# mstksg/tensor-ops

Measured on AMD Instinct MI355X. Metric: gradTOp steps/sec (ffLayer MNIST 784->256->10) + gmul TFLOP/s vs roofline, higher is better.
Workload: dtype f32

## Files before the change

### tensor-ops_amd/csrc/gemm_t32.hip

```cpp
#include <cstdio>
#include <type_traits>

#include "common.hpp"
#include "arg_fit.hpp"

namespace to {

typedef float f32x16 __attribute__((ext_vector_type(16)));
typedef float f32x4 __attribute__((ext_vector_type(4)));

struct T32Args {
  const float* A;
  const float* B;
  long a_sx, b_sx;
  int M, N, K;
  int tiles_m, tiles_n;
  int lgm, lgn;
  unsigned wmag0, wmag1;
  int pd;
  float* C;
  const float* Cin;
  const float* bias;
  const float* dact;
  float* rowsum;
  const float* rowsum_in;
  unsigned long long* dbg;
  long c_sm;
  int gm, gn;
  int act, dact_kind;
  int rowsum_acc;
  float alpha, beta;
  float rowsum_alpha;
};

__device__ __forceinline__ void t32_pin_hot(const T32Args& g) {
  asm volatile("" ::"s"(g.A), "s"(g.B), "s"(g.a_sx), "s"(g.b_sx), "s"(g.M), "s"(g.N), "s"(g.K), "s"(g.tiles_m), "s"(g.tiles_n),
               "s"(g.lgm), "s"(g.lgn), "s"(g.wmag0), "s"(g.wmag1), "s"(g.pd));
}

__device__ __attribute__((aligned(16))) float g_t32_zero[4] = {0.f, 0.f, 0.f, 0.f};

constexpr int T32_BK = 32, T32_NS = 2, T32_NW = 4;
constexpr int T32_CTR = 4096;
constexpr int T32_STAGE = 2 * 32 * T32_BK;
constexpr int T32_WAVE = T32_NS * T32_STAGE;

__device__ __forceinline__ bool t32_tile_of(const T32Args& g, int bid, int& tm, int& tn) {
  const int x = bid & 7, local = bid >> 3, xm = x >> g.lgn, xn = x & ((1 << g.lgn) - 1);
  const int r0 = (g.tiles_m * xm) >> g.lgm, r1 = (g.tiles_m * (xm + 1)) >> g.lgm;
  const int c0 = (g.tiles_n * xn) >> g.lgn, c1 = (g.tiles_n * (xn + 1)) >> g.lgn;
  const int w = c1 - c0;
  if (w <= 0 || local >= (r1 - r0) * w) return false;
  const unsigned mag = w == (g.tiles_n >> g.lgn) ? g.wmag0 : g.wmag1;
  const int q = w == 1 ? local : (int)__umulhi((unsigned)local, mag);
  tm = r0 + q;
  tn = c0 + local - q * w;
  return true;
}

__device__ __forceinline__ int t32_key(int x) { return (x >> 1) & 7; }

template <bool AKC, bool BKC, bool ARAG = false, bool WT = false, int NW = T32_NW, int NS = T32_NS, bool EARLY = false, bool REGU = false, bool PIN = true>
__device__ __forceinline__ int gemm_t32_body(const T32Args& g, const int bid, float* smem) {
  static_assert(!REGU || (NW == 8 && NS == 1 && EARLY && !ARAG), "the register unit belongs to the eight-wave, one-stage, early-DMA form");
  constexpr int WAVE_F = NS * T32_STAGE;
  static_assert(WAVE_F >= 1024 + 64, "a wave's stage memory holds its partial tile and its row sums");
  static_assert(!ARAG || !AKC, "the dword form is for a row-contiguous A");
  constexpr int NA = ARAG ? 16 : 4, PER = NA + 4;
#ifdef TOPS_AB_KNOBS
  const unsigned long long t_entry = __builtin_amdgcn_s_memrealtime();
#endif
  if constexpr (PIN) t32_pin_hot(g);
  const int tid = threadIdx.x, lane = tid & 63;
  const int wave = __builtin_amdgcn_readfirstlane(tid >> 6);
  const int l31 = lane & 31, half = lane >> 5;
#ifdef TOPS_AB_KNOBS
  unsigned long long* dbg = nullptr;
  unsigned long long* wdbg = nullptr;
  auto stamp = [&](int i) { if (dbg) dbg[i] = __builtin_amdgcn_s_memrealtime(); };
  auto stamp_first = [&] {
    const bool mine = g.dbg && (bid == 0 || bid == (int)gridDim.x - 1);
    dbg = (mine && tid == 0) ? g.dbg + (bid == 0 ? 0 : 8) : nullptr;
    wdbg = (mine && lane == 0 && wave < 8) ? g.dbg + 16 + (bid == 0 ? 0 : 16) + 2 * wave : nullptr;
    if (dbg) { dbg[0] = t_entry; dbg[6] = __builtin_amdgcn_s_memrealtime(); }
  };
#else
  auto stamp = [](int) {};
  auto stamp_first = [] {};
#endif
#ifdef TOPS_AB_KNOBS
#define T32_WSTAMP(i) do { if (wdbg) wdbg[i] = __builtin_amdgcn_s_memrealtime(); } while (0)
#else
#define T32_WSTAMP(i) do { } while (0)
#endif
  int tile_m, tile_n;
  if (!t32_tile_of(g, bid, tile_m, tile_n)) return -1;
  const int m0 = tile_m * 32, n0 = tile_n * 32;

  const int erow = tid >> 3, ec4 = (tid & 7) * 4;
  const long grow = m0 + erow, gcol = n0 + ec4;
  const bool evalid = (NW == 4 || tid < 256) && grow < g.M && gcol < g.N;
  f32x4 pf_ci = {0.f, 0.f, 0.f, 0.f}, pf_hd = {0.f, 0.f, 0.f, 0.f}, pf_bias = {0.f, 0.f, 0.f, 0.f};
  auto prefetch_epilogue = [&] {
    if (evalid) {
      if (g.Cin) pf_ci = *reinterpret_cast<const f32x4*>(g.Cin + grow * g.c_sm + gcol);
      if (g.dact) pf_hd = *reinterpret_cast<const f32x4*>(g.dact + grow * g.c_sm + gcol);
      if (g.bias) pf_bias = *reinterpret_cast<const f32x4*>(g.bias + gcol);
    }
  };
  if constexpr (!EARLY) prefetch_epilogue();

  const int U = (g.K + 15) / 16;
  const int k0 = (int)((unsigned)(U * wave) / (unsigned)NW) * 16;
  int k1 = (int)((unsigned)(U * (wave + 1)) / (unsigned)NW) * 16;
  if (k1 > g.K) k1 = g.K;
  int kd = k1;
  bool ru = false;
  if constexpr (REGU) {
    const int nU = (k1 - k0 + 15) / 16;
    ru = (nU & 1) != 0;
    if (ru) kd = k0 + (nU - 1) * 16;
  }
  const int nC = kd > k0 ? (kd - k0 + T32_BK - 1) / T32_BK : 0;

  typedef __attribute__((address_space(3))) void* lptr_t;
  float* wsm = smem + wave * WAVE_F;
  const unsigned lds_w = __builtin_amdgcn_readfirstlane((unsigned)(unsigned long)(lptr_t)wsm);

  const int lr = lane >> 3, ls = lane & 7;
  unsigned oa[4], ob[4];
  bool xa_ok = true, xb_ok = true;
#pragma unroll
  for (int p = 0; p < 4; ++p) {
    if constexpr (AKC) {
      long x = m0 + 8 * p + lr;
      if (x >= g.M) x = g.M - 1;
      oa[p] = (unsigned)((x * g.a_sx + 4 * (ls ^ t32_key(8 * p + lr))) * 4);
    } else {
      oa[p] = (unsigned)(((long)(8 * p + lr) * g.a_sx + m0 + 4 * ls) * 4);
    }
    if constexpr (BKC) {
      long x = n0 + 8 * p + lr;
      if (x >= g.N) x = g.N - 1;
      ob[p] = (unsigned)((x * g.b_sx + 4 * (ls ^ t32_key(8 * p + lr))) * 4);
    } else {
      ob[p] = (unsigned)(((long)(8 * p + lr) * g.b_sx + n0 + 4 * ls) * 4);
    }
  }
  if constexpr (!AKC) xa_ok = m0 + 4 * ls + 3 < g.M;
  if constexpr (!BKC) xb_ok = n0 + 4 * ls + 3 < g.N;
  const bool interior = !ARAG && (AKC || m0 + 32 <= g.M) && (BKC || n0 + 32 <= g.N);
  const long step_a = AKC ? T32_BK * 4L : T32_BK * g.a_sx * 4L, step_b = BKC ? T32_BK * 4L : T32_BK * g.b_sx * 4L;
  const char* sa = reinterpret_cast<const char*>(g.A) + (AKC ? (long)k0 * 4 : (long)k0 * g.a_sx * 4);
  const char* sb = reinterpret_cast<const char*>(g.B) + (BKC ? (long)k0 * 4 : (long)k0 * g.b_sx * 4);

#define T32_DMA(OFF, BASE) asm volatile("global_load_lds_dwordx4 %0, %1 offset:0" ::"v"(OFF), "s"(BASE) : "memory")
#define T32_DMA_V(PTR) asm volatile("global_load_lds_dwordx4 %0, off offset:0" ::"v"(PTR) : "memory")
  const long a_sx_l = g.a_sx;
  const int M_l = g.M;
  auto issue = [&, a_sx_l, M_l](int c) {
    const int seq = c;
    const int kc = k0 + c * T32_BK;
    const unsigned st = lds_w + (unsigned)(seq % NS) * (T32_STAGE * 4);
    const char* ba = sa + (long)c * step_a;
    const char* bb = sb + (long)c * step_b;
    const bool full = kc + T32_BK <= kd;
    if (full && interior) {
#pragma unroll
      for (int p = 0; p < 4; ++p) {
        asm volatile("s_mov_b32 m0, %0\n\ts_nop 0" ::"s"(st + p * 1024) : "memory");
        T32_DMA(oa[p], ba);
      }
#pragma unroll
      for (int p = 0; p < 4; ++p) {
        asm volatile("s_mov_b32 m0, %0\n\ts_nop 0" ::"s"(st + 4096 + p * 1024) : "memory");
        T32_DMA(ob[p], bb);
      }
    } else {
      const char* zero = reinterpret_cast<const char*>(g_t32_zero);
      if constexpr (ARAG) {
#pragma unroll
        for (int e = 0; e < 16; ++e) {
          const int kl = 2 * e + half;
          const bool ok = kc + kl < kd && m0 + l31 < M_l;
          const char* src = ok ? ba + ((long)kl * a_sx_l + m0 + l31) * 4 : zero;
          asm volatile("s_mov_b32 m0, %0\n\ts_nop 0" ::"s"(st + e * 256) : "memory");
          asm volatile("global_load_lds_dword %0, off offset:0" ::"v"(src) : "memory");
        }
      } else {
#pragma unroll
        for (int p = 0; p < 4; ++p) {
          const bool ok = AKC ? (kc + 4 * (ls ^ t32_key(8 * p + lr)) < kd) : (kc + 8 * p + lr < kd && xa_ok);
          const char* src = ok ? ba + oa[p] : zero;
          asm volatile("s_mov_b32 m0, %0\n\ts_nop 0" ::"s"(st + p * 1024) : "memory");
          T32_DMA_V(src);
        }
      }
#pragma unroll
      for (int p = 0; p < 4; ++p) {
        const bool ok = BKC ? (kc + 4 * (ls ^ t32_key(8 * p + lr)) < kd) : (kc + 8 * p + lr < kd && xb_ok);
        const char* src = ok ? bb + ob[p] : zero;
        asm volatile("s_mov_b32 m0, %0\n\ts_nop 0" ::"s"(st + 4096 + p * 1024) : "memory");
        T32_DMA_V(src);
      }
    }
  };
#undef T32_DMA
#undef T32_DMA_V

  f32x16 acc;
#pragma unroll
  for (int r = 0; r < 16; ++r) acc[r] = 0.f;
  float asum = 0.f;
  bool want_rs;

  const int PD = g.pd < NS ? g.pd : NS;
  const int pro = nC < PD ? nC : PD;
  f32x4 ua4[2], ub4[2];
  float ua1[8], ub1[8];
  if constexpr (REGU) {
    if (ru) {
      const float* zero = g_t32_zero;
#pragma unroll
      for (int i = 0; i < 2; ++i) {
        const int kq = kd + 4 * (2 * i + half);
        if constexpr (AKC) {
          long x = m0 + l31;
          if (x >= g.M) x = g.M - 1;
          const float* src = kq < k1 ? g.A + x * g.a_sx + kq : zero;
          asm volatile("global_load_dwordx4 %0, %1, off" : "=&v"(ua4[i]) : "v"(src) : "memory");
        } else {
#pragma unroll
          for (int j = 0; j < 4; ++j) {
            const float* src = (kq + j < k1 && m0 + l31 < g.M) ? g.A + (long)(kq + j) * g.a_sx + m0 + l31 : zero;
            asm volatile("global_load_dword %0, %1, off" : "=&v"(ua1[4 * i + j]) : "v"(src) : "memory");
          }
        }
        if constexpr (BKC) {
          long x = n0 + l31;
          if (x >= g.N) x = g.N - 1;
          const float* src = kq < k1 ? g.B + x * g.b_sx + kq : zero;
          asm volatile("global_load_dwordx4 %0, %1, off" : "=&v"(ub4[i]) : "v"(src) : "memory");
        } else {
#pragma unroll
          for (int j = 0; j < 4; ++j) {
            const float* src = (kq + j < k1 && n0 + l31 < g.N) ? g.B + (long)(kq + j) * g.b_sx + n0 + l31 : zero;
            asm volatile("global_load_dword %0, %1, off" : "=&v"(ub1[4 * i + j]) : "v"(src) : "memory");
          }
        }
      }
    }
    __builtin_amdgcn_sched_barrier(0);
  }
  if constexpr (EARLY) {
    if (pro > 0) issue(0);
    __builtin_amdgcn_sched_barrier(0);
    stamp_first();
    want_rs = g.rowsum != nullptr && tile_n == 0;
    if constexpr (REGU) {
      if (ru) {
        if (pro > 0) asm volatile("s_waitcnt vmcnt(%0)" ::"n"(PER) : "memory");
        else asm volatile("s_waitcnt vmcnt(0)" ::: "memory");
        float fu[8], gu[8];
        if constexpr (AKC) {
          asm volatile("" : "+v"(ua4[0]), "+v"(ua4[1]) :: "memory");
#pragma unroll
          for (int i = 0; i < 2; ++i) { fu[4 * i] = ua4[i].x; fu[4 * i + 1] = ua4[i].y; fu[4 * i + 2] = ua4[i].z; fu[4 * i + 3] = ua4[i].w; }
        } else {
          asm volatile("" : "+v"(ua1[0]), "+v"(ua1[1]), "+v"(ua1[2]), "+v"(ua1[3]), "+v"(ua1[4]), "+v"(ua1[5]), "+v"(ua1[6]), "+v"(ua1[7]) :: "memory");
#pragma unroll
          for (int q = 0; q < 8; ++q) fu[q] = ua1[q];
        }
        if constexpr (BKC) {
          asm volatile("" : "+v"(ub4[0]), "+v"(ub4[1]) :: "memory");
#pragma unroll
          for (int i = 0; i < 2; ++i) { gu[4 * i] = ub4[i].x; gu[4 * i + 1] = ub4[i].y; gu[4 * i + 2] = ub4[i].z; gu[4 * i + 3] = ub4[i].w; }
        } else {
          asm volatile("" : "+v"(ub1[0]), "+v"(ub1[1]), "+v"(ub1[2]), "+v"(ub1[3]), "+v"(ub1[4]), "+v"(ub1[5]), "+v"(ub1[6]), "+v"(ub1[7]) :: "memory");
#pragma unroll
          for (int q = 0; q < 8; ++q) gu[q] = ub1[q];
        }
        __builtin_amdgcn_sched_barrier(0);
#pragma unroll
        for (int q = 0; q < 8; ++q) {
          acc = __builtin_amdgcn_mfma_f32_32x32x2f32(fu[q], gu[q], acc, 0, 0, 0);
          if (want_rs) asum += fu[q];
        }
      }
      __builtin_amdgcn_sched_barrier(0);
    }
    prefetch_epilogue();
    __builtin_amdgcn_sched_barrier(0);
    for (int c = 1; c < pro; ++c) issue(c);
  } else {
    for (int c = 0; c < pro; ++c) issue(c);
    stamp_first();
    want_rs = g.rowsum != nullptr && tile_n == 0;
  }
  stamp(1);

  auto wait_landed = [&](int c) {
    const int newer = (nC - 1 - c) < (PD - 1) ? (nC - 1 - c) : (PD - 1);
    static_assert(3 * PER <= 63, "vmcnt is six bits");
    if (newer >= 3) asm volatile("s_waitcnt vmcnt(%0)" ::"n"(3 * PER) : "memory");
    else if (newer == 2) asm volatile("s_waitcnt vmcnt(%0)" ::"n"(2 * PER) : "memory");
    else if (newer == 1) asm volatile("s_waitcnt vmcnt(%0)" ::"n"(PER) : "memory");
    else asm volatile("s_waitcnt vmcnt(0)" ::: "memory");
  };
  auto steps_of = [&](int c) { return (kd - (k0 + c * T32_BK)) > 16 ? 4 : 2; };
  auto read_frags = [&](int c, float (&fa)[16], float (&fb)[16]) {
    const float* sp = wsm + (c % NS) * T32_STAGE;
    const int nI = steps_of(c);
#pragma unroll
    for (int i = 0; i < 4; ++i) {
      if (i < nI) {
        if constexpr (AKC) {
          const f32x4 v = *reinterpret_cast<const f32x4*>(sp + l31 * 32 + 4 * ((2 * i + half) ^ t32_key(l31)));
          fa[4 * i] = v.x; fa[4 * i + 1] = v.y; fa[4 * i + 2] = v.z; fa[4 * i + 3] = v.w;
        } else {
#pragma unroll
          for (int j = 0; j < 4; ++j) fa[4 * i + j] = sp[(4 * (2 * i + half) + j) * 32 + l31];
        }
        if constexpr (BKC) {
          const f32x4 v = *reinterpret_cast<const f32x4*>(sp + 1024 + l31 * 32 + 4 * ((2 * i + half) ^ t32_key(l31)));
          fb[4 * i] = v.x; fb[4 * i + 1] = v.y; fb[4 * i + 2] = v.z; fb[4 * i + 3] = v.w;
        } else {
#pragma unroll
          for (int j = 0; j < 4; ++j) fb[4 * i + j] = sp[1024 + (4 * (2 * i + half) + j) * 32 + l31];
        }
      }
    }
  };
  auto mma = [&](int c, const float (&fa)[16], const float (&fb)[16]) {
    const int nI = steps_of(c);
#pragma unroll
    for (int i = 0; i < 4; ++i) {
      if (i < nI) {
#pragma unroll
        for (int j = 0; j < 4; ++j) {
          acc = __builtin_amdgcn_mfma_f32_32x32x2f32(fa[4 * i + j], fb[4 * i + j], acc, 0, 0, 0);
          if (want_rs) asum += fa[4 * i + j];
        }
      }
    }
  };
  float fa[16], fb[16];
  for (int c = 0; c < nC; ++c) {
    wait_landed(c);
    if (c == 0) stamp(2);
    read_frags(c, fa, fb);
    asm volatile("s_waitcnt lgkmcnt(0)" ::: "memory");
    __builtin_amdgcn_sched_barrier(0);
    if (c + PD < nC) issue(c + PD);
    __builtin_amdgcn_sched_barrier(0);
    mma(c, fa, fb);
  }
  asm volatile("s_waitcnt vmcnt(0)" ::: "memory");
  stamp(3);
  T32_WSTAMP(0);

#pragma unroll
  for (int r = 0; r < 16; ++r) wsm[((r & 3) + 8 * (r >> 2) + 4 * half) * 32 + l31] = acc[r];
  if (want_rs) wsm[1024 + lane] = asum;
  T32_WSTAMP(1);
  __syncthreads();
  stamp(4);
  f32x4 s = {0.f, 0.f, 0.f, 0.f};
  if (NW == 4 || tid < 256) {
    s = *reinterpret_cast<const f32x4*>(smem + erow * 32 + ec4);
#pragma unroll
    for (int w = 1; w < NW; ++w) s += *reinterpret_cast<const f32x4*>(smem + w * WAVE_F + erow * 32 + ec4);
  }
  if (evalid) {
    f32x4 v = s * g.alpha;
    if (g.Cin) v += pf_ci * g.beta;
    if (g.bias) v += pf_bias;
    if (g.act == 1) {
      v.x = 1.f / (1.f + __expf(-v.x)); v.y = 1.f / (1.f + __expf(-v.y));
      v.z = 1.f / (1.f + __expf(-v.z)); v.w = 1.f / (1.f + __expf(-v.w));
    } else if (g.act == 2) {
      v.x = tanhf(v.x); v.y = tanhf(v.y); v.z = tanhf(v.z); v.w = tanhf(v.w);
    }
    if (g.dact) {
      if (g.dact_kind == 0) v *= pf_hd * (1.f - pf_hd);
      else v *= 1.f - pf_hd * pf_hd;
    }
    if constexpr (WT) {
      typedef unsigned int u32x4 __attribute__((ext_vector_type(4)));
      const u32x4 u = {__float_as_uint(v.x), __float_as_uint(v.y), __float_as_uint(v.z), __float_as_uint(v.w)};
      float* dst = g.C + grow * g.c_sm + gcol;
      asm volatile("global_store_dwordx4 %0, %1, off sc0 sc1" ::"v"(dst), "v"(u) : "memory");
    } else {
      *reinterpret_cast<f32x4*>(g.C + grow * g.c_sm + gcol) = v;
    }
  }
  if (want_rs && tid < 32) {
    const long m = m0 + tid;
    if (m < g.M) {
      float t = 0.f;
#pragma unroll
      for (int w = 0; w < NW; ++w) t += smem[w * WAVE_F + 1024 + tid] + smem[w * WAVE_F + 1024 + 32 + tid];
      if (g.rowsum_acc) g.rowsum[m] = (g.rowsum_in ? g.rowsum_in[m] : g.rowsum[m]) + g.rowsum_alpha * t;
      else g.rowsum[m] = t;
    }
  }
  stamp(5);
#undef T32_WSTAMP
  return tile_m;
}

struct T32HeadArgs {
  const float* W2;
  const float* bias2;
  const float* target;
  float* dz;
  float* loss_out;
  float* tail_out;
  unsigned* ctr;
  int* status;
  long w_sn, dz_sm;
  int N2, loss_rows;
  float alpha2;
};

__global__ __launch_bounds__(256) void gemm_t32_head_kernel(T32Args g, T32HeadArgs h) {
  extern __shared__ __attribute__((aligned(1024))) float t32_smem[];
  const int tid = threadIdx.x, lane = tid & 63;
  const int wave = __builtin_amdgcn_readfirstlane(tid >> 6);
  const unsigned long long t_entry = g.dbg ? __builtin_amdgcn_s_memrealtime() : 0ull;
  int tile_m, tile_n;
  if (!t32_tile_of(g, (int)blockIdx.x, tile_m, tile_n)) return;
  const long grow = (long)tile_m * 32 + 4 * tile_n + wave;
  const bool rv = grow < g.M;
  f32x4 w4[16];
#pragma unroll
  for (int n = 0; n < 16; ++n) {
    w4[n] = f32x4{0.f, 0.f, 0.f, 0.f};
    if (n < h.N2) w4[n] = *reinterpret_cast<const f32x4*>(h.W2 + (long)n * h.w_sn + 4 * lane);
  }
  const float b_l = (lane < h.N2 && h.bias2) ? h.bias2[lane] : 0.f;
  const float t_l = (lane < h.N2 && rv) ? h.target[grow * h.dz_sm + lane] : 0.f;

  gemm_t32_body<true, true, false, true>(g, (int)blockIdx.x, t32_smem);

  unsigned long long* const hd = (g.dbg && tid == 0 && blockIdx.x == 0) ? g.dbg + 8 : nullptr;
  asm volatile("s_waitcnt vmcnt(0)" ::: "memory");
  __syncthreads();
  __shared__ int gave_up;
  if (tid == 0) {
    unsigned* arrive = h.ctr + tile_m;
    __hip_atomic_fetch_add(arrive, 1u, __ATOMIC_RELAXED, __HIP_MEMORY_SCOPE_AGENT);
    if (hd) { hd[0] = t_entry; hd[1] = __builtin_amdgcn_s_memrealtime(); hd[7] = 1; }
    const unsigned long long t0 = __builtin_amdgcn_s_memrealtime();
    int bad = 0;
    while (__hip_atomic_load(arrive, __ATOMIC_RELAXED, __HIP_MEMORY_SCOPE_AGENT) < (unsigned)g.tiles_n) {
      __builtin_amdgcn_s_sleep(2);
      if (__builtin_amdgcn_s_memrealtime() - t0 > 200000000ull) {
        bad = 1;
        break;
      }
    }
    gave_up = bad;
    if (bad && h.status) *h.status = tile_m + 1;
  }
  __syncthreads();
  if (gave_up) return;
  if (hd) hd[2] = __builtin_amdgcn_s_memrealtime();

  typedef unsigned int u32x4 __attribute__((ext_vector_type(4)));
  f32x4 h4 = {0.f, 0.f, 0.f, 0.f};
  if (rv) {
    u32x4 u;
    const float* src = g.C + grow * g.c_sm + 4 * lane;
    asm volatile("global_load_dwordx4 %0, %1, off sc0 sc1\n\ts_waitcnt vmcnt(0)" : "=v"(u) : "v"(src) : "memory");
    h4 = f32x4{__uint_as_float(u.x), __uint_as_float(u.y), __uint_as_float(u.z), __uint_as_float(u.w)};
  }
  float z[16];
#pragma unroll
  for (int n = 0; n < 16; ++n) {
    z[n] = 0.f;
    if (n < h.N2) {
      z[n] = h4.x * w4[n].x + h4.y * w4[n].y + h4.z * w4[n].z + h4.w * w4[n].w;
#pragma unroll
      for (int off = 1; off < 64; off <<= 1) z[n] += __shfl_xor(z[n], off, 64);
    }
  }
  float v = -INFINITY;
#pragma unroll
  for (int n = 0; n < 16; ++n)
    if (n < h.N2 && lane == n) v = z[n] * h.alpha2 + b_l;
  auto sum16 = [](float x) {
#pragma unroll
    for (int off = 8; off > 0; off >>= 1) x += __shfl_xor(x, off, 64);
    return x;
  };
  const bool lv = lane < h.N2;
  float out_l, loss_l;
  if (h.loss_rows == 1) {
    float mx = v;
#pragma unroll
    for (int off = 8; off > 0; off >>= 1) mx = fmaxf(mx, __shfl_xor(mx, off, 64));
    const float e = lv ? expf(v - mx) : 0.f;
    const float se = sum16(e), sy = sum16(t_l);
    const float pr = e / se;
    out_l = lv ? pr * sy - t_l : 0.f;
    loss_l = lv ? -t_l * logf(pr) : 0.f;
  } else {
    const float sg = 1.f / (1.f + expf(-v));
    const float e = t_l - sg;
    out_l = lv ? -2.f * e * sg * (1.f - sg) : 0.f;
    loss_l = lv ? e * e : 0.f;
  }
  if (rv) {
    if (lv) h.dz[grow * h.dz_sm + lane] = out_l;
    if (h.loss_out) {
      const float l = sum16(loss_l);
      if (lane == 0) h.loss_out[grow] = l;
    }
  }
  if (hd) hd[3] = __builtin_amdgcn_s_memrealtime();
  if (h.tail_out) {
    f32x4 a = {0.f, 0.f, 0.f, 0.f};
#pragma unroll
    for (int n = 0; n < 16; ++n)
      if (n < h.N2) {
        const float d = __shfl(out_l, n, 64);
        a += w4[n] * d;
      }
    if (rv) *reinterpret_cast<f32x4*>(h.tail_out + grow * 256 + 4 * lane) = a * h4 * (1.f - h4);
  }
  if (hd) hd[4] = __builtin_amdgcn_s_memrealtime();
  __syncthreads();
  if (tid == 0) {
    unsigned* leave = h.ctr + T32_CTR + tile_m;
    const unsigned seen = __hip_atomic_fetch_add(leave, 1u, __ATOMIC_RELAXED, __HIP_MEMORY_SCOPE_AGENT);
    if (seen == (unsigned)(g.tiles_n - 1)) {
      __hip_atomic_store(h.ctr + tile_m, 0u, __ATOMIC_RELAXED, __HIP_MEMORY_SCOPE_AGENT);
      __hip_atomic_store(leave, 0u, __ATOMIC_RELAXED, __HIP_MEMORY_SCOPE_AGENT);
    }
  }
}

__host__ __device__ __forceinline__ int t32_tiles(int extent) { return (extent + 31) >> 5; }
__host__ __device__ __forceinline__ unsigned t32_pack_map(int lgm, int lgn, int pd) { return (unsigned)lgm | ((unsigned)lgn << 8) | ((unsigned)pd << 16); }

template <bool AKC, bool BKC, int NW = T32_NW, int NS = T32_NS, bool EARLY = false, bool REGU = false>
__global__ __launch_bounds__(NW * 64) void gemm_t32_kernel(const float* A, const float* B, int a_sx, int b_sx, int M, int N, int K,
                                                           unsigned map, unsigned wmag0, unsigned wmag1, T32Args cold) {
  extern __shared__ __attribute__((aligned(1024))) float t32_smem[];
  T32Args g = cold;
  g.A = A; g.B = B;
  g.a_sx = a_sx; g.b_sx = b_sx;
  g.M = M; g.N = N; g.K = K;
  g.tiles_m = t32_tiles(M); g.tiles_n = t32_tiles(N);
  g.lgm = (int)(map & 255u); g.lgn = (int)((map >> 8) & 255u); g.pd = (int)(map >> 16);
  g.wmag0 = wmag0; g.wmag1 = wmag1;
  gemm_t32_body<AKC, BKC, false, false, NW, NS, EARLY, REGU, false>(g, (int)blockIdx.x, t32_smem);
}

template <bool ARAG2>
__global__ __launch_bounds__(256) void gemm_t32_pair_kernel(T32Args g1, T32Args g2, int n1) {
  extern __shared__ __attribute__((aligned(1024))) float t32_smem[];
  if ((int)blockIdx.x < n1) gemm_t32_body<false, false, false>(g1, (int)blockIdx.x, t32_smem);
  else gemm_t32_body<false, false, ARAG2>(g2, (int)blockIdx.x - n1, t32_smem);
}

static bool t32_plan_map(T32Args& g) {
  if ((long)g.tiles_m * g.tiles_n > 65535) return false;
  auto lg = [](int v) { int l = 0; while ((1 << l) < v) ++l; return l; };
  auto mag = [](int w) { return w >= 2 ? (unsigned)((0xFFFFFFFFull / (unsigned)w) + 1ull) : 0u; };
  g.lgm = lg(g.gm);
  g.lgn = lg(g.gn);
  const int wlo = g.tiles_n >> g.lgn;
  g.wmag0 = mag(wlo);
  g.wmag1 = mag(wlo + 1);
  return true;
}

static bool t32_fill(const GemmProblem& p, T32Args& g, bool& akc, bool& bkc, bool allow_ragged_a = false, bool* ragged_a = nullptr) {
  if (p.dtype != TO_F32 || p.batch != 1 || p.reduce_batch) return false;
  if (p.loss_rows || p.tail_out || p.loss_out) return false;
  akc = p.a_sk == 1 && p.K > 1;
  bkc = p.b_sk == 1 && p.K > 1;
  if (!akc && p.a_sm != 1) return false;
  if (!bkc && p.b_sn != 1) return false;
  if (p.K % 4 != 0 || p.N % 4 != 0) return false;
  const bool rag = !akc && (p.M % 4 != 0 || p.a_sk % 4 != 0 || (reinterpret_cast<uintptr_t>(p.A) & 15u));
  if (ragged_a) *ragged_a = rag;
  if (rag && !allow_ragged_a) return false;
  if (akc && p.a_sm % 4 != 0) return false;
  if (bkc && p.b_sn % 4 != 0) return false;
  if (!bkc && p.b_sk % 4 != 0) return false;
  if ((reinterpret_cast<uintptr_t>(p.A) & 3u) || ((akc || !rag) && (reinterpret_cast<uintptr_t>(p.A) & 15u))) return false;
  if ((reinterpret_cast<uintptr_t>(p.B) | reinterpret_cast<uintptr_t>(p.C)) & 15u) return false;
  if (p.c_sm % 4 != 0) return false;
  if (p.Cin && (reinterpret_cast<uintptr_t>(p.Cin) & 15u)) return false;
  if (p.dact && (reinterpret_cast<uintptr_t>(p.dact) & 15u)) return false;
  if (p.bias && (reinterpret_cast<uintptr_t>(p.bias) & 15u)) return false;
  if (p.beta != 0.0 && !p.Cin) return false;
  if (p.act > 2) return false;
  if (!t32_spans_fit(p.M, p.N, p.K, p.a_sm, p.a_sk, p.b_sn, p.b_sk)) return false;
  g.A = (const float*)p.A; g.B = (const float*)p.B; g.C = (float*)p.C;
  g.Cin = p.beta != 0.0 ? (const float*)p.Cin : nullptr;
  g.M = (int)p.M; g.N = (int)p.N; g.K = (int)p.K;
  g.a_sx = akc ? p.a_sm : p.a_sk;
  g.b_sx = bkc ? p.b_sn : p.b_sk;
  g.c_sm = p.c_sm;
  g.tiles_m = t32_tiles((int)p.M); g.tiles_n = t32_tiles((int)p.N);
  {
    int best = 1 << 30;
    for (int gm : {8, 4, 2, 1}) {
      const int gn = 8 / gm;
      const int cost = (g.tiles_m + gm - 1) / gm + (g.tiles_n + gn - 1) / gn;
      if (cost < best) { best = cost; g.gm = gm; g.gn = gn; }
    }
  }
  if (!t32_plan_map(g)) return false;
  g.alpha = (float)p.alpha; g.beta = (float)p.beta;
  g.bias = (const float*)p.bias; g.dact = (const float*)p.dact; g.act = p.act; g.dact_kind = p.dact_kind;
  g.rowsum = (float*)p.rowsum; g.rowsum_in = (const float*)p.rowsum_in; g.rowsum_alpha = (float)p.rowsum_alpha;
  g.rowsum_acc = p.rowsum_acc ? 1 : 0;
  static const int pd = [] { const char* e = ab_getenv("TOPS_T32_PD"); const int v = e ? atoi(e) : 2; return v < 1 ? 1 : (v > T32_NS ? T32_NS : v); }();
  g.pd = pd;
  static unsigned long long* dbg = [] {
    unsigned long long* p = nullptr;
    if (ab_getenv("TOPS_T32_STAMPS") && hipHostMalloc(reinterpret_cast<void**>(&p), 48 * sizeof(unsigned long long), hipHostMallocMapped) == hipSuccess) {
      for (int i = 0; i < 48; ++i) p[i] = 0;
      static unsigned long long* keep = p;
      atexit([] {
        if (keep[15]) {
          const unsigned long long* k = keep + 8;
          std::fprintf(stderr, "[t32] joined launch, workgroup 0, us since it began: its tile stored and arrived %.2f, all eight tiles of the row block "
                               "there %.2f, loss head of its four rows done %.2f, tail stored %.2f (entered %.2f us after stamp 0)\n",
                       (k[1] - k[0]) * 0.01, (k[2] - k[0]) * 0.01, (k[3] - k[0]) * 0.01, (k[4] - k[0]) * 0.01, ((double)k[0] - (double)keep[0]) * 0.01);
        }
        for (int w = 0; w < (keep[15] ? 1 : 2); ++w) {
          const unsigned long long* k = keep + 8 * w;
          std::fprintf(stderr, "[t32] %s workgroup of the last launch, us since its first instruction: first operand load out %.2f, prologue DMA issued %.2f, "
                               "first chunk landed %.2f, K loop done %.2f, partials met %.2f, done %.2f; began %.2f us after workgroup 0\n", w ? "last" : "first",
                       (k[6] - k[0]) * 0.01, (k[1] - k[0]) * 0.01, (k[2] - k[0]) * 0.01, (k[3] - k[0]) * 0.01, (k[4] - k[0]) * 0.01, (k[5] - k[0]) * 0.01,
                       ((double)k[0] - (double)keep[0]) * 0.01);
          const unsigned long long* wv = keep + 16 + 16 * w;
          std::fprintf(stderr, "[t32]   per wave, K loop done / partial written:");
          for (int q = 0; q < 8; ++q)
            if (wv[2 * q]) std::fprintf(stderr, "  w%d %.2f / %.2f", q, ((double)wv[2 * q] - (double)k[0]) * 0.01, ((double)wv[2 * q + 1] - (double)k[0]) * 0.01);
          std::fprintf(stderr, "\n");
        }
      });
    }
    return p;
  }();
  g.dbg = dbg;
  return true;
}

bool gemm_t32_applicable(const GemmProblem& p) {
  static const int enable = [] { const char* e = ab_getenv("TOPS_GEMM_T32"); return e ? atoi(e) : 1; }();
  if (!enable) return false;
  T32Args g;
  bool akc, bkc;
  if (!t32_fill(p, g, akc, bkc)) return false;
  const long tiles = (long)g.tiles_m * g.tiles_n;
  static const long max_tiles = [] { const char* e = ab_getenv("TOPS_T32_MAXTILES"); return e ? atol(e) : 512L; }();
  return tiles >= 96 && tiles <= max_tiles && p.K >= 256 && p.K <= 8192;
}

bool launch_gemm_t32_pair(const GemmProblem& p1, const GemmProblem& p2, hipStream_t s, bool dry);

static long t32_grid(const T32Args& g) {
  const long rm = (g.tiles_m + g.gm - 1) / g.gm, rn = (g.tiles_n + g.gn - 1) / g.gn;
  return 8 * rm * rn;
}

static void t32_attr(const void* k) { TO_HIP(hipFuncSetAttribute(k, hipFuncAttributeMaxDynamicSharedMemorySize, T32_NW * T32_WAVE * 4)); }

constexpr int T32_W8_DEFAULT = 1;
constexpr int T32_W8_NS = 1;
constexpr bool T32_EARLY = true;
constexpr bool T32_REGU = true;

template <int NW, int NS, bool EARLY, bool REGU = false>
static void t32_launch_nw(const T32Args& g, bool akc, bool bkc, hipStream_t s) {
  constexpr size_t lds = (size_t)NW * NS * T32_STAGE * 4;
  static bool attr = false;
  if (!attr) {
    TO_HIP(hipFuncSetAttribute(reinterpret_cast<const void*>(gemm_t32_kernel<true, true, NW, NS, EARLY, REGU>), hipFuncAttributeMaxDynamicSharedMemorySize, (int)lds));
    TO_HIP(hipFuncSetAttribute(reinterpret_cast<const void*>(gemm_t32_kernel<true, false, NW, NS, EARLY, REGU>), hipFuncAttributeMaxDynamicSharedMemorySize, (int)lds));
    TO_HIP(hipFuncSetAttribute(reinterpret_cast<const void*>(gemm_t32_kernel<false, true, NW, NS, EARLY, REGU>), hipFuncAttributeMaxDynamicSharedMemorySize, (int)lds));
    TO_HIP(hipFuncSetAttribute(reinterpret_cast<const void*>(gemm_t32_kernel<false, false, NW, NS, EARLY, REGU>), hipFuncAttributeMaxDynamicSharedMemorySize, (int)lds));
    attr = true;
  }
  const dim3 grid((unsigned)t32_grid(g)), block(NW * 64);
#define T32_HOT g.A, g.B, (int)g.a_sx, (int)g.b_sx, g.M, g.N, g.K, t32_pack_map(g.lgm, g.lgn, g.pd), g.wmag0, g.wmag1
  if (akc && bkc) launch_k((gemm_t32_kernel<true, true, NW, NS, EARLY, REGU>), grid, block, lds, s, T32_HOT, g);
  else if (akc) launch_k((gemm_t32_kernel<true, false, NW, NS, EARLY, REGU>), grid, block, lds, s, T32_HOT, g);
  else if (bkc) launch_k((gemm_t32_kernel<false, true, NW, NS, EARLY, REGU>), grid, block, lds, s, T32_HOT, g);
  else launch_k((gemm_t32_kernel<false, false, NW, NS, EARLY, REGU>), grid, block, lds, s, T32_HOT, g);
#undef T32_HOT
}

void launch_gemm_t32(const GemmProblem& p, hipStream_t s) {
  T32Args g;
  bool akc, bkc;
  TO_CHECK(t32_fill(p, g, akc, bkc), TO_ERR_STATE, "launch_gemm_t32: not applicable");
  static const int cus = [] { hipDeviceProp_t pr; int d = 0; return (hipGetDevice(&d) == hipSuccess && hipGetDeviceProperties(&pr, d) == hipSuccess) ? pr.multiProcessorCount : 0; }();
  static const int waves = [] { const char* e = ab_getenv("TOPS_T32_WAVES"); return e ? atoi(e) : (T32_W8_DEFAULT ? 8 : 4); }();
  const bool w8 = waves == 8 && t32_grid(g) <= cus;
#ifdef TOPS_AB_KNOBS
  static const int w8_ns = [] { const char* e = ab_getenv("TOPS_T32_W8_NS"); return e ? atoi(e) : T32_W8_NS; }();
  static const int early = [] { const char* e = ab_getenv("TOPS_T32_EARLY"); return e ? atoi(e) : (int)T32_EARLY; }();
  static const int regu = [] { const char* e = ab_getenv("TOPS_T32_REGU"); return e ? atoi(e) : (int)T32_REGU; }();
  switch ((w8 ? (w8_ns == 1 ? 2 : 4) : 0) + (early ? 1 : 0)) {
    case 0: t32_launch_nw<T32_NW, T32_NS, false>(g, akc, bkc, s); break;
    case 1: t32_launch_nw<T32_NW, T32_NS, true>(g, akc, bkc, s); break;
    case 2: t32_launch_nw<8, 1, false>(g, akc, bkc, s); break;
    case 3:
      if (regu) t32_launch_nw<8, 1, true, true>(g, akc, bkc, s);
      else t32_launch_nw<8, 1, true, false>(g, akc, bkc, s);
      break;
    case 4: t32_launch_nw<8, 2, false>(g, akc, bkc, s); break;
    default: t32_launch_nw<8, 2, true>(g, akc, bkc, s); break;
  }
#else
  if (w8) t32_launch_nw<8, T32_W8_NS, T32_EARLY, T32_REGU>(g, akc, bkc, s);
  else t32_launch_nw<T32_NW, T32_NS, T32_EARLY>(g, akc, bkc, s);
#endif
  TO_HIP(hipGetLastError());
  count_launch();
}

static unsigned* g_t32_ctr = nullptr;
static int *g_t32_status = nullptr, *g_t32_status_dev = nullptr;
static bool g_t32_head_off = false;
void gemm_t32_init() {
  if (g_t32_ctr) return;
  if (hipMalloc(&g_t32_ctr, 2 * T32_CTR * sizeof(unsigned)) != hipSuccess || hipMemset(g_t32_ctr, 0, 2 * T32_CTR * sizeof(unsigned)) != hipSuccess) {
    (void)hipGetLastError();
    g_t32_ctr = nullptr;
    return;
  }
  if (hipHostMalloc(&g_t32_status, sizeof(int), hipHostMallocMapped) == hipSuccess) {
    *g_t32_status = 0;
    if (hipHostGetDevicePointer(reinterpret_cast<void**>(&g_t32_status_dev), g_t32_status, 0) != hipSuccess) g_t32_status_dev = nullptr;
  }
  (void)hipGetLastError();
}
int gemm_t32_take_failure() {
  const int st = g_t32_status ? *g_t32_status : 0;
  if (st) {
    g_t32_head_off = true;
    *g_t32_status = 0;
    if (g_t32_ctr) (void)hipMemset(g_t32_ctr, 0, 2 * T32_CTR * sizeof(unsigned));
  }
  return st;
}

bool launch_gemm_t32_head(const GemmProblem& pf, const GemmProblem& ph, hipStream_t s) {
  static const int enable = [] { const char* e = getenv("TOPS_STEP_SEAM"); return e ? atoi(e) : 0; }();
  if (enable != 3 || !g_t32_ctr || !g_t32_status_dev || g_t32_head_off) return false;
  T32Args g;
  bool akc, bkc;
  if (!t32_fill(pf, g, akc, bkc) || !akc || !bkc) return false;
  const long tiles = (long)g.tiles_m * g.tiles_n;
  if (tiles < 96 || tiles > 512 || pf.K < 256 || pf.K > 8192 || g.tiles_m > T32_CTR) return false;
  if (pf.act != 1 || pf.dact || pf.rowsum || pf.beta != 0.0) return false;
  if (pf.N != 256 || pf.c_sm != pf.N) return false;
  if (ph.dtype != TO_F32 || ph.batch != 1 || ph.reduce_batch) return false;
  if (ph.A != pf.C || ph.M != pf.M || ph.K != pf.N || ph.a_sk != 1 || ph.a_sm != pf.c_sm) return false;
  if (ph.b_sk != 1 || ph.b_sn % 4 != 0 || (reinterpret_cast<uintptr_t>(ph.B) & 15u)) return false;
  if (ph.N < 1 || ph.N > 16 || (ph.loss_rows != 1 && ph.loss_rows != 2) || !ph.target) return false;
  if (ph.beta != 0.0 || ph.dact || ph.act != 0 || ph.rowsum) return false;
  if (ph.tail_out) {
    if (ph.tail_kind) return false;
    if (ph.tail_n != pf.N || ph.tail_h != pf.C || ph.tail_w != ph.B || ph.b_sn != ph.tail_n) return false;
    if (reinterpret_cast<uintptr_t>(ph.tail_out) & 15u) return false;
  }
  g.gm = 8; g.gn = 1;
  if (!t32_plan_map(g)) return false;
  if (g.tiles_m < 8) return false;
  {
    static const int cus = [] { hipDeviceProp_t pr; int d = 0; return (hipGetDevice(&d) == hipSuccess && hipGetDeviceProperties(&pr, d) == hipSuccess) ? pr.multiProcessorCount : 0; }();
    if (t32_grid(g) > cus) return false;
  }
  T32HeadArgs h{};
  h.W2 = (const float*)ph.B; h.bias2 = (const float*)ph.bias; h.target = (const float*)ph.target;
  h.dz = (float*)ph.C; h.loss_out = (float*)ph.loss_out; h.tail_out = (float*)ph.tail_out;
  h.ctr = g_t32_ctr;
  h.status = g_t32_status_dev;
  h.w_sn = ph.b_sn; h.dz_sm = ph.c_sm;
  h.N2 = (int)ph.N; h.loss_rows = ph.loss_rows; h.alpha2 = (float)ph.alpha;

  static bool attr = false;
  if (!attr) {
    TO_HIP(hipFuncSetAttribute(reinterpret_cast<const void*>(gemm_t32_head_kernel), hipFuncAttributeMaxDynamicSharedMemorySize, T32_NW * T32_WAVE * 4));
    attr = true;
  }
  launch_k(gemm_t32_head_kernel, dim3((unsigned)t32_grid(g)), dim3(256), (size_t)T32_NW * T32_WAVE * 4, s, g, h);
  TO_HIP(hipGetLastError());
  count_launch();
  return true;
}

bool launch_gemm_t32_pair(const GemmProblem& p1, const GemmProblem& p2, hipStream_t s, bool dry) {
  static const int enable = [] { const char* e = ab_getenv("TOPS_GEMM_T32_PAIR"); return e ? atoi(e) : 0; }();
  if (!enable) return false;
  T32Args g1, g2;
  bool akc1, bkc1, akc2, bkc2, rag2 = false;
  if (!t32_fill(p1, g1, akc1, bkc1) || akc1 || bkc1) return false;
  if (!t32_fill(p2, g2, akc2, bkc2, true, &rag2) || akc2 || bkc2) return false;
  const long n1 = (long)g1.tiles_m * g1.tiles_n, n2 = (long)g2.tiles_m * g2.tiles_n;
  if (n1 < 96 || n1 + n2 > 512 || p1.K < 256 || p1.K > 8192 || p2.K < 256 || p2.K > 8192 || n2 > n1) return false;
  if (dry) return true;
  static bool attr = false;
  if (!attr) {
    t32_attr(reinterpret_cast<const void*>(gemm_t32_pair_kernel<false>));
    t32_attr(reinterpret_cast<const void*>(gemm_t32_pair_kernel<true>));
    attr = true;
  }
  const long w1 = t32_grid(g1), w2 = t32_grid(g2);
  const dim3 grid((unsigned)(w1 + w2)), block(256);
  const size_t lds = (size_t)T32_NW * T32_WAVE * 4;
  if (rag2) launch_k(gemm_t32_pair_kernel<true>, grid, block, lds, s, g1, g2, (int)w1);
  else launch_k(gemm_t32_pair_kernel<false>, grid, block, lds, s, g1, g2, (int)w1);
  TO_HIP(hipGetLastError());
  count_launch();
  return true;
}

}
```

Baseline: 48330.

## Restructure register-unit GEMM path into variable-size K trips with 16-wide sub-chunks

```diff
diff --git a/tensor-ops_amd/csrc/gemm_t32.hip b/tensor-ops_amd/csrc/gemm_t32.hip
--- a/tensor-ops_amd/csrc/gemm_t32.hip
+++ b/tensor-ops_amd/csrc/gemm_t32.hip
@@ -3,6 +3,7 @@
 
 #include "common.hpp"
 #include "arg_fit.hpp"
+#include "t32_trips.hpp"
 
 namespace to {
 
@@ -59,12 +60,23 @@
 }
 
 __device__ __forceinline__ int t32_key(int x) { return (x >> 1) & 7; }
+__device__ __forceinline__ int t32_key16(int x) { return (x >> 2) & 3; }
 
 template <bool AKC, bool BKC, bool ARAG = false, bool WT = false, int NW = T32_NW, int NS = T32_NS, bool EARLY = false, bool REGU = false, bool PIN = true>
 __device__ __forceinline__ int gemm_t32_body(const T32Args& g, const int bid, float* smem) {
   static_assert(!REGU || (NW == 8 && NS == 1 && EARLY && !ARAG), "the register unit belongs to the eight-wave, one-stage, early-DMA form");
-  constexpr int WAVE_F = NS * T32_STAGE;
-  static_assert(WAVE_F >= 1024 + 64, "a wave's stage memory holds its partial tile and its row sums");
+#ifdef TOPS_AB_KNOBS
+  const int trip_s = REGU ? ((g.pd >> 8) & 15) : 0, trip_lead = REGU ? ((g.pd >> 12) & 15) : 0;
+  constexpr int QMAX = T32_TRIP_SMAX;
+  constexpr bool FIRST2 = false, ALL2 = false;
+#else
+  constexpr int trip_s = T32_TRIP_S, trip_lead = T32_TRIP_LEAD;
+  constexpr int QMAX = T32_TRIP_S;
+  constexpr bool FIRST2 = t32_trips_first_is_pair(T32_TRIP_S, T32_TRIP_LEAD), ALL2 = t32_trips_all_pairs(T32_TRIP_S, T32_TRIP_LEAD);
+#endif
+  static_assert(QMAX <= T32_TRIP_SMAX && 4 * T32_TRIP_SMAX <= 63, "a trip's DMA instructions are counted in vmcnt: six bits");
+  const int WAVE_F = REGU ? trip_s * 1024 : NS * T32_STAGE;
+  static_assert(NS * T32_STAGE >= 1024 + 64 && T32_TRIP_S >= 2, "a wave's stage memory holds its partial tile and its row sums");
   static_assert(!ARAG || !AKC, "the dword form is for a row-contiguous A");
   constexpr int NA = ARAG ? 16 : 4, PER = NA + 4;
 #ifdef TOPS_AB_KNOBS
@@ -122,6 +134,9 @@
     if (ru) kd = k0 + (nU - 1) * 16;
   }
   const int nC = kd > k0 ? (kd - k0 + T32_BK - 1) / T32_BK : 0;
+  const int nD = REGU ? (kd - k0 + 15) >> 4 : 0;
+  const int nT = !REGU ? 0 : ALL2 ? nD >> 1 : t32_trip_count(nD, trip_s, trip_lead);
+  const int u0 = !(REGU && nT > 0) ? 0 : FIRST2 ? 2 : t32_trip_units(nD, trip_s, 0, trip_lead);
 
   typedef __attribute__((address_space(3))) void* lptr_t;
   float* wsm = smem + wave * WAVE_F;
@@ -147,6 +162,24 @@
       ob[p] = (unsigned)(((long)(8 * p + lr) * g.b_sx + n0 + 4 * ls) * 4);
     }
   }
+  unsigned oa16[2] = {0u, 0u}, ob16[2] = {0u, 0u};
+  auto offsets16 = [&] {
+#pragma unroll
+    for (int p = 0; p < 2; ++p) {
+      const int xr = 16 * p + (lane >> 2), qs = (lane & 3) ^ t32_key16(xr);
+      if constexpr (AKC) {
+        long x = m0 + xr;
+        if (x >= g.M) x = g.M - 1;
+        oa16[p] = (unsigned)((x * g.a_sx + 4 * qs) * 4);
+      }
+      if constexpr (BKC) {
+        long x = n0 + xr;
+        if (x >= g.N) x = g.N - 1;
+        ob16[p] = (unsigned)((x * g.b_sx + 4 * qs) * 4);
+      }
+    }
+  };
+  if constexpr (REGU && !FIRST2) offsets16();
   if constexpr (!AKC) xa_ok = m0 + 4 * ls + 3 < g.M;
   if constexpr (!BKC) xb_ok = n0 + 4 * ls + 3 < g.N;
   const bool interior = !ARAG && (AKC || m0 + 32 <= g.M) && (BKC || n0 + 32 <= g.N);
@@ -158,12 +191,7 @@
 #define T32_DMA_V(PTR) asm volatile("global_load_lds_dwordx4 %0, off offset:0" ::"v"(PTR) : "memory")
   const long a_sx_l = g.a_sx;
   const int M_l = g.M;
-  auto issue = [&, a_sx_l, M_l](int c) {
-    const int seq = c;
-    const int kc = k0 + c * T32_BK;
-    const unsigned st = lds_w + (unsigned)(seq % NS) * (T32_STAGE * 4);
-    const char* ba = sa + (long)c * step_a;
-    const char* bb = sb + (long)c * step_b;
+  auto issue32 = [&, a_sx_l, M_l](const int kc, const char* ba, const char* bb, const unsigned st) {
     const bool full = kc + T32_BK <= kd;
     if (full && interior) {
 #pragma unroll
@@ -204,6 +232,47 @@
         T32_DMA_V(src);
       }
     }
+  };
+  auto issue = [&](int c) {
+    issue32(k0 + c * T32_BK, sa + (long)c * step_a, sb + (long)c * step_b, lds_w + (unsigned)(c % NS) * (T32_STAGE * 4));
+  };
+  auto issue16 = [&](const int kc, const char* ba, const char* bb, const unsigned st) {
+    if (kc + 16 <= kd && interior) {
+#pragma unroll
+      for (int p = 0; p < 2; ++p) {
+        asm volatile("s_mov_b32 m0, %0\n\ts_nop 0" ::"s"(st + p * 1024) : "memory");
+        T32_DMA(AKC ? oa16[p] : oa[p], ba);
+      }
+#pragma unroll
+      for (int p = 0; p < 2; ++p) {
+        asm volatile("s_mov_b32 m0, %0\n\ts_nop 0" ::"s"(st + 2048 + p * 1024) : "memory");
+        T32_DMA(BKC ? ob16[p] : ob[p], bb);
+      }
+    } else {
+      const char* zero = reinterpret_cast<const char*>(g_t32_zero);
+#pragma unroll
+      for (int p = 0; p < 2; ++p) {
+        const bool ok = AKC ? (kc + 4 * ((lane & 3) ^ t32_key16(16 * p + (lane >> 2))) < kd) : (kc + 8 * p + lr < kd && xa_ok);
+        const char* src = ok ? ba + (AKC ? oa16[p] : oa[p]) : zero;
+        asm volatile("s_mov_b32 m0, %0\n\ts_nop 0" ::"s"(st + p * 1024) : "memory");
+        T32_DMA_V(src);
+      }
+#pragma unroll
+      for (int p = 0; p < 2; ++p) {
+        const bool ok = BKC ? (kc + 4 * ((lane & 3) ^ t32_key16(16 * p + (lane >> 2))) < kd) : (kc + 8 * p + lr < kd && xb_ok);
+        const char* src = ok ? bb + (BKC ? ob16[p] : ob[p]) : zero;
+        asm volatile("s_mov_b32 m0, %0\n\ts_nop 0" ::"s"(st + 2048 + p * 1024) : "memory");
+        T32_DMA_V(src);
+      }
+    }
+  };
+  auto issue_trip = [&](const int ub, const int u) {
+    int q = 0;
+#pragma nounroll
+    for (; q + 2 <= u; q += 2)
+      issue32(k0 + (ub + q) * 16, sa + (long)(ub + q) * (step_a / 2), sb + (long)(ub + q) * (step_b / 2), lds_w + (unsigned)q * 4096u);
+    if constexpr (!ALL2)
+      if (q < u) issue16(k0 + (ub + q) * 16, sa + (long)(ub + q) * (step_a / 2), sb + (long)(ub + q) * (step_b / 2), lds_w + (unsigned)q * 4096u);
   };
 #undef T32_DMA
 #undef T32_DMA_V
@@ -253,13 +322,20 @@
     __builtin_amdgcn_sched_barrier(0);
   }
   if constexpr (EARLY) {
-    if (pro > 0) issue(0);
+    if constexpr (REGU) {
+      if (nT > 0) issue_trip(0, u0);
+    } else {
+      if (pro > 0) issue(0);
+    }
     __builtin_amdgcn_sched_barrier(0);
     stamp_first();
     want_rs = g.rowsum != nullptr && tile_n == 0;
     if constexpr (REGU) {
       if (ru) {
-        if (pro > 0) asm volatile("s_waitcnt vmcnt(%0)" ::"n"(PER) : "memory");
+        if (u0 >= 4) asm volatile("s_waitcnt vmcnt(16)" ::: "memory");
+        else if (u0 == 3) asm volatile("s_waitcnt vmcnt(12)" ::: "memory");
+        else if (u0 == 2) asm volatile("s_waitcnt vmcnt(8)" ::: "memory");
+        else if (u0 == 1) asm volatile("s_waitcnt vmcnt(4)" ::: "memory");
         else asm volatile("s_waitcnt vmcnt(0)" ::: "memory");
         float fu[8], gu[8];
         if constexpr (AKC) {
@@ -291,6 +367,7 @@
     }
     prefetch_epilogue();
     __builtin_amdgcn_sched_barrier(0);
+    if constexpr (REGU && FIRST2 && !ALL2) offsets16();
     for (int c = 1; c < pro; ++c) issue(c);
   } else {
     for (int c = 0; c < pro; ++c) issue(c);
@@ -344,16 +421,68 @@
       }
     }
   };
-  float fa[16], fb[16];
-  for (int c = 0; c < nC; ++c) {
-    wait_landed(c);
-    if (c == 0) stamp(2);
-    read_frags(c, fa, fb);
-    asm volatile("s_waitcnt lgkmcnt(0)" ::: "memory");
-    __builtin_amdgcn_sched_barrier(0);
-    if (c + PD < nC) issue(c + PD);
-    __builtin_amdgcn_sched_barrier(0);
-    mma(c, fa, fb);
+  if constexpr (REGU) {
+    float fa[8 * QMAX], fb[8 * QMAX];
+    int ub = 0, u = u0;
+    for (int t = 0; t < nT; ++t) {
+      asm volatile("s_waitcnt vmcnt(0)" ::: "memory");
+      if (t == 0) stamp(2);
+#pragma unroll
+      for (int q = 0; q < QMAX; ++q) {
+        if (q < u) {
+          const bool in32 = ALL2 || (q & 1) || q + 1 < u;
+#pragma unroll
+          for (int ii = 0; ii < 2; ++ii) {
+            const int kq = 2 * (2 * (q & 1) + ii) + half;
+            const float* a32 = wsm + (q >> 1) * 2048;
+            const float* a16 = wsm + q * 1024;
+            if constexpr (AKC) {
+              const f32x4 v = *reinterpret_cast<const f32x4*>(in32 ? a32 + l31 * 32 + 4 * (kq ^ t32_key(l31)) : a16 + l31 * 16 + 4 * ((2 * ii + half) ^ t32_key16(l31)));
+              fa[8 * q + 4 * ii] = v.x; fa[8 * q + 4 * ii + 1] = v.y; fa[8 * q + 4 * ii + 2] = v.z; fa[8 * q + 4 * ii + 3] = v.w;
+            } else {
+#pragma unroll
+              for (int j = 0; j < 4; ++j) fa[8 * q + 4 * ii + j] = *(in32 ? a32 + (4 * kq + j) * 32 + l31 : a16 + (4 * (2 * ii + half) + j) * 32 + l31);
+            }
+            if constexpr (BKC) {
+              const f32x4 v = *reinterpret_cast<const f32x4*>(in32 ? a32 + 1024 + l31 * 32 + 4 * (kq ^ t32_key(l31)) : a16 + 512 + l31 * 16 + 4 * ((2 * ii + half) ^ t32_key16(l31)));
+              fb[8 * q + 4 * ii] = v.x; fb[8 * q + 4 * ii + 1] = v.y; fb[8 * q + 4 * ii + 2] = v.z; fb[8 * q + 4 * ii + 3] = v.w;
+            } else {
+#pragma unroll
+              for (int j = 0; j < 4; ++j) fb[8 * q + 4 * ii + j] = *(in32 ? a32 + 1024 + (4 * kq + j) * 32 + l31 : a16 + 512 + (4 * (2 * ii + half) + j) * 32 + l31);
+            }
+          }
+        }
+      }
+      asm volatile("s_waitcnt lgkmcnt(0)" ::: "memory");
+      __builtin_amdgcn_sched_barrier(0);
+      const int un = t + 1 >= nT ? 0 : ALL2 ? 2 : t32_trip_units(nD, trip_s, t + 1, trip_lead);
+      if (un > 0) issue_trip(ub + u, un);
+      __builtin_amdgcn_sched_barrier(0);
+#pragma unroll
+      for (int q = 0; q < QMAX; ++q) {
+        if (q < u) {
+#pragma unroll
+          for (int s = 0; s < 8; ++s) {
+            acc = __builtin_amdgcn_mfma_f32_32x32x2f32(fa[8 * q + s], fb[8 * q + s], acc, 0, 0, 0);
+            if (want_rs) asum += fa[8 * q + s];
+          }
+        }
+      }
+      ub += u;
+      u = un;
+    }
+  } else {
+    float fa[16], fb[16];
+    for (int c = 0; c < nC; ++c) {
+      wait_landed(c);
+      if (c == 0) stamp(2);
+      read_frags(c, fa, fb);
+      asm volatile("s_waitcnt lgkmcnt(0)" ::: "memory");
+      __builtin_amdgcn_sched_barrier(0);
+      if (c + PD < nC) issue(c + PD);
+      __builtin_amdgcn_sched_barrier(0);
+      mma(c, fa, fb);
+    }
   }
   asm volatile("s_waitcnt vmcnt(0)" ::: "memory");
   stamp(3);
@@ -679,9 +808,22 @@
 constexpr bool T32_EARLY = true;
 constexpr bool T32_REGU = true;
 
+static int t32_trip_bits() {
+  static const int bits = [] {
+    const char* e = ab_getenv("TOPS_T32_TRIPS");
+    const int v = e ? atoi(e) : 0;
+    int S = T32_TRIP_S, lead = T32_TRIP_LEAD;
+    if (v == 24) { S = 4; lead = 2; }
+    else if (v >= 2 && v <= T32_TRIP_SMAX) { S = v; lead = 0; }
+    return S | (lead << 4);
+  }();
+  return bits;
+}
+
 template <int NW, int NS, bool EARLY, bool REGU = false>
 static void t32_launch_nw(const T32Args& g, bool akc, bool bkc, hipStream_t s) {
-  constexpr size_t lds = (size_t)NW * NS * T32_STAGE * 4;
+  const int trips = REGU ? t32_trip_bits() : 0;
+  const size_t lds = REGU ? (size_t)t32_trip_lds_bytes(trips & 15) : (size_t)NW * NS * T32_STAGE * 4;
   static bool attr = false;
   if (!attr) {
     TO_HIP(hipFuncSetAttribute(reinterpret_cast<const void*>(gemm_t32_kernel<true, true, NW, NS, EARLY, REGU>), hipFuncAttributeMaxDynamicSharedMemorySize, (int)lds));
@@ -691,7 +833,7 @@
     attr = true;
   }
   const dim3 grid((unsigned)t32_grid(g)), block(NW * 64);
-#define T32_HOT g.A, g.B, (int)g.a_sx, (int)g.b_sx, g.M, g.N, g.K, t32_pack_map(g.lgm, g.lgn, g.pd), g.wmag0, g.wmag1
+#define T32_HOT g.A, g.B, (int)g.a_sx, (int)g.b_sx, g.M, g.N, g.K, t32_pack_map(g.lgm, g.lgn, g.pd | (trips << 8)), g.wmag0, g.wmag1
   if (akc && bkc) launch_k((gemm_t32_kernel<true, true, NW, NS, EARLY, REGU>), grid, block, lds, s, T32_HOT, g);
   else if (akc) launch_k((gemm_t32_kernel<true, false, NW, NS, EARLY, REGU>), grid, block, lds, s, T32_HOT, g);
   else if (bkc) launch_k((gemm_t32_kernel<false, true, NW, NS, EARLY, REGU>), grid, block, lds, s, T32_HOT, g);
diff --git a/tensor-ops_amd/csrc/t32_trips.hpp b/tensor-ops_amd/csrc/t32_trips.hpp
--- /dev/null
+++ b/tensor-ops_amd/csrc/t32_trips.hpp
@@ -0,0 +1,54 @@
+#pragma once
+
+#if defined(__HIPCC__) || defined(__CUDACC__)
+#define T32_TRIP_HD __host__ __device__ inline
+#else
+#define T32_TRIP_HD inline
+#endif
+
+namespace to {
+
+constexpr int T32_TRIP_SMAX = 4;
+#ifndef TOPS_T32_TRIP_S
+#define TOPS_T32_TRIP_S 2
+#endif
+#ifndef TOPS_T32_TRIP_LEAD
+#define TOPS_T32_TRIP_LEAD 0
+#endif
+constexpr int T32_TRIP_S = TOPS_T32_TRIP_S;
+constexpr int T32_TRIP_LEAD = TOPS_T32_TRIP_LEAD;
+static_assert(T32_TRIP_S >= 2 && T32_TRIP_S <= T32_TRIP_SMAX && T32_TRIP_LEAD >= 0 && T32_TRIP_LEAD <= T32_TRIP_S, "the stage holds every trip");
+
+constexpr bool t32_trips_first_is_pair(int S, int lead) { return lead > 0 ? lead == 2 : S == 2; }
+constexpr bool t32_trips_all_pairs(int S, int lead) { return S == 2 && (lead == 0 || lead == 2); }
+
+T32_TRIP_HD int t32_ceil_div_stage(int n, int S) {
+  switch (S) {
+    case 1: return n;
+    case 2: return (n + 1) / 2;
+    case 3: return (n + 2) / 3;
+    default: return (n + 3) / 4;
+  }
+}
+
+T32_TRIP_HD int t32_trip_count(int n, int S, int lead = 0) {
+  if (n <= 0) return 0;
+  if (lead > 0 && n > lead) return 1 + t32_ceil_div_stage(n - lead, S);
+  return t32_ceil_div_stage(n, S);
+}
+
+T32_TRIP_HD int t32_trip_units(int n, int S, int t, int lead = 0) {
+  if (lead > 0 && n > lead) {
+    if (t == 0) return lead;
+    n -= lead;
+    --t;
+  }
+  const int T = t32_ceil_div_stage(n, S);
+  int q = 0;
+  for (int c = 1; c <= T32_TRIP_SMAX; ++c) q += (c <= S && c * T <= n) ? 1 : 0;
+  return q + (t < n - q * T ? 1 : 0);
+}
+
+T32_TRIP_HD int t32_trip_lds_bytes(int S) { return 8 * S * 4096; }
+
+}
```

Result: no change. 48310 (-0.0%).
